# sukui-genomics-cn/hmm_layer

Hardware: AMD Instinct MI355X
Metric: HMM cell-updates/sec (batch x len x states) fwd-bwd, 15-state model (higher is better)
Workload: dtype f32

## Files before the change

### hmm_layer_amd/csrc/hmm_engine.hip

```cpp

#include <hip/hip_runtime.h>
#include <stdint.h>
#include <stdlib.h>
#include <mutex>
#include <type_traits>
#include <vector>
#include "hmm_engine.h"

typedef float f4 __attribute__((ext_vector_type(4)));
typedef int i4 __attribute__((ext_vector_type(4)));

#ifndef HMM_REDUCE_PF
#define HMM_REDUCE_PF 8
#endif
#ifndef HMM_NT_STORE
#define HMM_NT_STORE 1
#endif
#ifndef HMM_PSI
#define HMM_PSI 1
#endif
#ifndef HMM_BWD_FULL
#define HMM_BWD_FULL 0
#endif
#ifndef HMM_FWD_PF2
// ... 158 lines not shown
    f4 d = __builtin_amdgcn_mfma_f32_16x16x4f32(a[0], x.x, z, 0, 0, 0);
    d = __builtin_amdgcn_mfma_f32_16x16x4f32(a[1], x.y, d, 0, 0, 0);
    d = __builtin_amdgcn_mfma_f32_16x16x4f32(a[2], x.z, d, 0, 0, 0);
    d = __builtin_amdgcn_mfma_f32_16x16x4f32(a[3], x.w, d, 0, 0, 0);
    return d;
}

__device__ __forceinline__ f4 mfma4v(f4 a, f4 x, f4 c) {
    c = __builtin_amdgcn_mfma_f32_16x16x4f32(a.x, x.x, c, 0, 0, 0);
    c = __builtin_amdgcn_mfma_f32_16x16x4f32(a.y, x.y, c, 0, 0, 0);
    c = __builtin_amdgcn_mfma_f32_16x16x4f32(a.z, x.z, c, 0, 0, 0);
    c = __builtin_amdgcn_mfma_f32_16x16x4f32(a.w, x.w, c, 0, 0, 0);
    return c;
}

__device__ __forceinline__ void swap16(float &a, float &b) {
    asm("s_nop 1\n\tv_permlane16_swap_b32_e32 %0, %1" : "+v"(a), "+v"(b));
}
__device__ __forceinline__ void swap32(float &a, float &b) {
    asm("s_nop 1\n\tv_permlane32_swap_b32_e32 %0, %1" : "+v"(a), "+v"(b));
}
__device__ __forceinline__ float col_sum(float v) {
    float a = v, b = v;
    swap16(a, b);
    a += b; b = a;
    swap32(a, b);
    return a + b;
}
__device__ __forceinline__ float col_max(float v) {
    float a = v, b = v;
    swap16(a, b);
    a = fmaxf(a, b); b = a;
    swap32(a, b);
    return fmaxf(a, b);
}
__device__ __forceinline__ float hsum(f4 v) { return (v.x + v.y) + (v.z + v.w); }
__device__ __forceinline__ float hmax(f4 v) { return fmaxf(fmaxf(v.x, v.y), fmaxf(v.z, v.w)); }

__device__ __forceinline__ __amdgpu_buffer_rsrc_t make_rsrc(const void *base, unsigned long long bytes) {
    unsigned n = bytes > 0xFFFFFFF0ull ? 0xFFFFFFF0u : (unsigned)bytes;
    return __builtin_amdgcn_make_buffer_rsrc((void *)base, 0, (int)n, 0x00020000);
}
template <int N>
__device__ __forceinline__ void ld_rows(__amdgpu_buffer_rsrc_t r, int voff, int rowb, f4 (&e)[N]) {
#pragma unroll
    for (int s = 0; s < N; ++s)
        e[s] = __builtin_bit_cast(f4, __builtin_amdgcn_raw_buffer_load_b128(r, voff + s * rowb, 0, HMM_LD_AUX));
}

struct Bounds { f4 lo, hi; };
__device__ __forceinline__ Bounds make_bounds(int g, int q, float eps) {
    Bounds bd;
    const float inf = __builtin_inff();
    bd.lo.x = (4 * g + 0 < q) ? eps : 0.f;  bd.hi.x = (4 * g + 0 < q) ? inf : 0.f;
    bd.lo.y = (4 * g + 1 < q) ? eps : 0.f;  bd.hi.y = (4 * g + 1 < q) ? inf : 0.f;
    bd.lo.z = (4 * g + 2 < q) ? eps : 0.f;  bd.hi.z = (4 * g + 2 < q) ? inf : 0.f;
    bd.lo.w = (4 * g + 3 < q) ? eps : 0.f;  bd.hi.w = (4 * g + 3 < q) ? inf : 0.f;
    return bd;
}
__device__ __forceinline__ f4 clampE(f4 e, const Bounds &bd) {
    f4 r;
    r.x = __builtin_amdgcn_fmed3f(e.x, bd.lo.x, bd.hi.x);
    r.y = __builtin_amdgcn_fmed3f(e.y, bd.lo.y, bd.hi.y);
    r.z = __builtin_amdgcn_fmed3f(e.z, bd.lo.z, bd.hi.z);
    r.w = __builtin_amdgcn_fmed3f(e.w, bd.lo.w, bd.hi.w);
    return r;
}
__device__ __forceinline__ f4 fmax4(f4 v, float s) {
    f4 r = {fmaxf(v.x, s), fmaxf(v.y, s), fmaxf(v.z, s), fmaxf(v.w, s)};
    return r;
}
__device__ __forceinline__ f4 sel4(bool c, f4 a, f4 b) { return c ? a : b; }

__device__ __forceinline__ void load_A(const float *A, int q, int g, int n, float (&af)[4], float (&ab)[4]) {
#pragma unroll
    for (int kk = 0; kk < 4; ++kk) {
        int s = 4 * g + kk;
        bool ok = (s < q) && (n < q);
        af[kk] = ok ? A[s * q + n] : 0.f;
        ab[kk] = ok ? A[n * q + s] : 0.f;
    }
}


__device__ __forceinline__ void reduce_chain(const float *__restrict__ A, const float *__restrict__ E,
                                             float *__restrict__ ops, int *__restrict__ exps,
                                             const int *__restrict__ topo, const Plan &p, float eps, long long chain) {
    const int lane = threadIdx.x & 63, g = lane >> 4, n = lane & 15;
    const int seq = (int)(chain / p.C), c = (int)(chain - (long long)seq * p.C);
    const int m = seq / p.b;
    if (topo && topo[m] != 0) return;
    const int t0 = c * p.T;
    const int len = min(p.T, p.L - t0);
    const int q = p.q;

    float af[4], ab[4];
    load_A(A + (size_t)m * q * q, q, g, n, af, ab);
    const Bounds bd = make_bounds(g, q, eps);

    const float *base = E + ((size_t)seq * p.L + t0) * q;
    const __amdgpu_buffer_rsrc_t rs = make_rsrc(base, (unsigned long long)len * q * sizeof(float));
    const int rowb = q * (int)sizeof(float);
    int voff = g * 16;

    f4 X;
    X.x = (4 * g + 0 == n) ? 1.f : 0.f;
    X.y = (4 * g + 1 == n) ? 1.f : 0.f;
    X.z = (4 * g + 2 == n) ? 1.f : 0.f;
    X.w = (4 * g + 3 == n) ? 1.f : 0.f;
    int ex = 0;

    auto rescale = [&](f4 &V) {
        float s = col_sum(hsum(V));
        int xe = __builtin_amdgcn_frexp_expf(s);
        float sc = __builtin_amdgcn_ldexpf(1.0f, -xe);
        V = V * sc;
        ex += xe;
    };

    int t = 0;
    if (c == 0 && p.seq_start) {
        f4 e0[1];
        ld_rows<1>(rs, voff, rowb, e0);
        X = X * clampE(e0[0], bd);
        rescale(X);
        voff += rowb;
        t = 1;
    }
    constexpr int PF = HMM_REDUCE_PF;
    f4 en[PF];
    ld_rows<PF>(rs, voff, rowb, en);
    for (; t < len; t += PF) {
        f4 ec[PF];
#pragma unroll
        for (int u = 0; u < PF; ++u) ec[u] = en[u];
        voff += PF * rowb;
        ld_rows<PF>(rs, voff, rowb, en);
#pragma unroll
        for (int u = 0; u < PF; ++u) {
            if (t + u < len) {
                X = mfma4(af, X) * clampE(ec[u], bd);
                rescale(X);
            }
        }
    }
    float *o = ops + (size_t)chain * QP * QP;
    o[(4 * g + 0) * QP + n] = X.x;
    o[(4 * g + 1) * QP + n] = X.y;
    o[(4 * g + 2) * QP + n] = X.z;
    o[(4 * g + 3) * QP + n] = X.w;
    if (g == 0) exps[(size_t)chain * QP + n] = ex;
}

__global__ __launch_bounds__(256) void k_reduce(const float *__restrict__ A, const float *__restrict__ E,
                                                float *__restrict__ ops, int *__restrict__ exps,
                                                const int *__restrict__ topo, Plan p, float eps) {
    const long long stride = (long long)gridDim.x * 4;
    for (long long chain = (long long)blockIdx.x * 4 + __builtin_amdgcn_readfirstlane(threadIdx.x >> 6);
         chain < p.nchains; chain += stride)
        reduce_chain(A, E, ops, exps, topo, p, eps, chain);
}



struct TopoGene15 {
    static constexpr int Q = 15, NE = 23, ID = 1;
    static constexpr int start[Q + 1] = {0, 2, 4, 6, 8, 10, 13, 15, 16, 17, 18, 19, 20, 21, 22, 23};
    static constexpr int src[NE] = {0, 14, 8, 1, 9, 2, 10, 3, 11, 6, 7, 4, 12, 5, 13, 0, 4, 5, 6, 1, 2, 3, 5};
};
struct TopoGene7 {
    static constexpr int Q = 7, NE = 15, ID = 2;
    static constexpr int start[Q + 1] = {0, 2, 4, 6, 8, 11, 13, 15};
    static constexpr int src[NE] = {0, 6, 4, 1, 5, 2, 6, 3, 0, 6, 3, 4, 1, 5, 2};
};

struct TopoGene29 {
    static constexpr int Q = 29, NE = 45, ID = 3;
    static constexpr int start[Q + 1] = {0, 3, 5, 7, 9, 11, 13, 15, 17, 19, 22, 25, 27, 29, 30, 31, 32, 33, 34, 35, 36,
                                         37, 38, 39, 40, 41, 42, 43, 44, 45};
    static constexpr int src[NE] = {0, 27, 28, 15, 1, 16, 2, 17, 3, 18, 4, 19, 5, 20, 6, 21, 11, 22, 12, 13, 7, 23, 14,
                                    8, 24, 9, 25, 10, 26, 0, 0, 7, 8, 9, 10, 11, 12, 1, 2, 3, 4, 5, 6, 9, 10};
};

template <class T>
__host__ __device__ constexpr int out_degree(int i) {
    int n = 0;
    for (int e = 0; e < T::NE; ++e) n += (T::src[e] == i) ? 1 : 0;
    return n;
}
#define TOPO_UNIT 16
template <class T>
__host__ __device__ constexpr bool passthrough(int j) {
    return T::start[j + 1] - T::start[j] == 1 && out_degree<T>(j) == 1;
}
template <class T>
__host__ __device__ constexpr int pt_src(int p) { return T::src[T::start[p]]; }
template <class T>
__host__ __device__ constexpr int pt_dst(int p) {
    for (int j = 0; j < T::Q; ++j)
        for (int e = T::start[j]; e < T::start[j + 1]; ++e)
            if (T::src[e] == p) return j;
    return -1;
}
template <class T>
__host__ __device__ constexpr int n_passthrough() {
    int n = 0;
    for (int j = 0; j < T::Q; ++j) n += passthrough<T>(j) ? 1 : 0;
    return n;
}
template <class T>
__host__ __device__ constexpr bool passthrough_between_live() {
    for (int p = 0; p < T::Q; ++p)
        if (passthrough<T>(p) && (passthrough<T>(pt_src<T>(p)) || passthrough<T>(pt_dst<T>(p)))) return false;
    return true;
}
static_assert(n_passthrough<TopoGene15>() == 8 && passthrough_between_live<TopoGene15>(), "15-state gene model: 7 live states");
static_assert(n_passthrough<TopoGene29>() == 16 && passthrough_between_live<TopoGene29>(), "29-state gene model: 13 live states");
static_assert(n_passthrough<TopoGene7>() == 0, "the 7-state model has no pass-through state");
template <class T>
__device__ __forceinline__ bool edge_in(int i, int j) {
    bool ok = false;
    for (int e = T::start[j]; e < T::start[j + 1]; ++e) ok = ok || (T::src[e] == i);
    return ok;
}

#define TOPO_EXACT 255
__global__ __launch_bounds__(64) void k_topo_check(const float *__restrict__ A, int *__restrict__ topo, int k, int q,
                                                   int force_dense, int exact_mode, float eps, int *__restrict__ nexact,
                                                   int *__restrict__ wcnt = nullptr) {
    const int m = blockIdx.x;
    const float *Am = A + (size_t)m * q * q;
    if (m == 0 && threadIdx.x == 0) *nexact = 0;
    if (m == 0 && threadIdx.x < 4 && wcnt) wcnt[threadIdx.x] = 0;
    bool exact = exact_mode == HMM_EXACT_ALWAYS || exact_mode == HMM_EXACT_ALWAYS_NARROW;
    if (exact_mode == HMM_EXACT_AUTO) {
        int row = 0;
        if ((int)threadIdx.x < q)
            for (int j = 0; j < q; ++j) row |= (Am[threadIdx.x * q + j] > eps) ? (1 << j) : 0;
        for (int it = 0; it < 8; ++it) {
            int nr = 0;
            for (int j = 0; j < q; ++j) {
                const int rj = __builtin_amdgcn_readlane(row, j);
                nr |= ((row >> j) & 1) ? rj : 0;
            }
            row = nr;
        }
        const bool notfull = (int)threadIdx.x < q && row != (1 << q) - 1;
        exact = __ballot(notfull) != 0ull;
    }
    if (exact) {
        if (threadIdx.x == 0) topo[m] = TOPO_EXACT;
        return;
    }
    bool bad15 = q != TopoGene15::Q, bad7 = q != TopoGene7::Q;
    bool nonunit15 = false, nonunit7 = false;
    if (!force_dense && (!bad15 || !bad7))
        for (int e = threadIdx.x; e < q * q; e += 64) {
            const float a = Am[e];
            const int i = e / q, j = e - i * q;
            if (!bad15) {
                const bool in = edge_in<TopoGene15>(i, j);
                bad15 = a != 0.f && !in;
                nonunit15 = nonunit15 || (in && a != 1.0f && out_degree<TopoGene15>(i) == 1);
            }
            if (!bad7) {
                const bool in = edge_in<TopoGene7>(i, j);
                bad7 = a != 0.f && !in;
                nonunit7 = nonunit7 || (in && a != 1.0f && out_degree<TopoGene7>(i) == 1);
            }
        }
    const bool any15 = __ballot(bad15) != 0ull, any7 = __ballot(bad7) != 0ull;
    const bool nu15 = __ballot(nonunit15) != 0ull, nu7 = __ballot(nonunit7) != 0ull;
    if (threadIdx.x == 0) {
        int id = force_dense ? 0 : (!any15 ? TopoGene15::ID : (!any7 ? TopoGene7::ID : 0));
        if (id == TopoGene15::ID && !nu15) id |= TOPO_UNIT;
        if (id == TopoGene7::ID && !nu7) id |= TOPO_UNIT;
        topo[m] = id;
    }
}

#define SP_TILE 16

#ifndef HMM_RS_AHEAD
#define HMM_RS_AHEAD 0
#endif
#ifndef HMM_RS_UNI
#define HMM_RS_UNI 1
#endif
#ifndef HMM_POST_BLOCK
#define HMM_POST_BLOCK 16
#endif
#ifndef HMM_RS_SUM2
#define HMM_RS_SUM2 1
#endif
#ifndef HMM_RS_ORDER2
#define HMM_RS_ORDER2 1
#endif
#ifndef HMM_RS_ROW128
#define HMM_RS_ROW128 1
#endif
#ifndef HMM_RS_WPE
#define HMM_RS_WPE 4
#endif
#if HMM_RS_WPE
#define RS_ATTR __attribute__((amdgpu_waves_per_eu(HMM_RS_WPE, HMM_RS_WPE)))
#else
#define RS_ATTR
#endif
template <class T> struct RsCfg {
    static constexpr int W = T::Q <= 16 ? 16 : 32;
    static constexpr int CPW = 64 / W;
    static constexpr int PIECES = SP_TILE * T::Q / 4;
    static constexpr int RPC = (PIECES + 63) / 64;
    typedef float Lds[2][CPW][SP_TILE * W + 16];
};

template <class T, bool UNIT, bool UNI>
__device__ __forceinline__ void reduce_sparse_wave(const float *__restrict__ A, const float *__restrict__ E,
                                                   float *__restrict__ ops, int *__restrict__ exps, const Plan &p,
                                                   float eps, typename RsCfg<T>::Lds &ldsw, long long wchain0,
                                                   bool mine, int m, long long chain, int c) {
    constexpr int Q = T::Q, W = RsCfg<T>::W, CPW = RsCfg<T>::CPW, RPC = RsCfg<T>::RPC;
    constexpr bool O2 = HMM_RS_ORDER2 && UNIT && UNI && n_passthrough<T>() > 0;
    static_assert(!O2 || passthrough_between_live<T>(), "a pass-through state between two live states");
    auto live = [](int j) constexpr { return !O2 || !passthrough<T>(j); };
    const int lane = threadIdx.x & 63, cl = lane / W, kc = lane % W;
    const int t0 = c * p.T;
    const int len = mine ? min(p.T, p.L - t0) : 0;
    const bool first = (c == 0) && p.seq_start;

    float a[T::NE];
    {
        const float *Am = A + (size_t)(UNI ? __builtin_amdgcn_readfirstlane(m) : m) * Q * Q;
#pragma unroll
        for (int j = 0; j < Q; ++j)
#pragma unroll
            for (int e = T::start[j]; e < T::start[j + 1]; ++e) a[e] = Am[T::src[e] * Q + j];
    }

    const int seq0 = (int)(wchain0 / p.C), c0 = (int)(wchain0 - (long long)seq0 * p.C);
    const long long row0 = (long long)seq0 * p.L + (long long)c0 * p.T;
    const unsigned long long total = (unsigned long long)p.NB * p.L * Q * sizeof(float);
    const __amdgpu_buffer_rsrc_t rs = make_rsrc(E + row0 * Q, total - (unsigned long long)row0 * Q * sizeof(float));
    constexpr int PIECES = RsCfg<T>::PIECES;
    static_assert(SP_TILE * Q % 4 == 0, "tile must be a whole number of 16-byte pieces");
    int coff[CPW];
#pragma unroll
    for (int j = 0; j < CPW; ++j) {
        long long ch = wchain0 + j;
        if (ch >= p.nchains) ch = wchain0;
        const long long sq = ch / p.C;
        const long long rw = sq * p.L + (ch - sq * p.C) * (long long)p.T;
        coff[j] = (int)((rw - row0) * Q * (long long)sizeof(float));
    }
    int loff[RPC][4];
#pragma unroll
    for (int rr = 0; rr < RPC; ++rr)
#pragma unroll
        for (int u = 0; u < 4; ++u) {
            const int idx = 4 * (rr * 64 + lane) + u;
            loff[rr][u] = (idx / Q) * W + (idx % Q);
        }
    float smul[O2 ? RPC : 1][4];
    if constexpr (O2) {
#pragma unroll
        for (int rr = 0; rr < RPC; ++rr)
#pragma unroll
            for (int u = 0; u < 4; ++u) {
                const int st = (4 * (rr * 64 + lane) + u) % Q;
                float mv = 1.f;
#pragma unroll
                for (int pp = 0; pp < Q; ++pp)
                    if (passthrough<T>(pp)) mv = (st == pp) ? a[T::start[pp]] : mv;
                smul[rr][u] = mv;
            }
    }
    for (int i = lane; i < 2 * CPW * (SP_TILE * W + 16); i += 64) (&ldsw[0][0][0])[i] = 0.f;

    f4 r[CPW * RPC];
    auto fetch = [&](int tile) {
#pragma unroll
        for (int j = 0; j < CPW; ++j)
#pragma unroll
            for (int rr = 0; rr < RPC; ++rr)
                r[j * RPC + rr] = __builtin_bit_cast(f4, __builtin_amdgcn_raw_buffer_load_b128(
                    rs, coff[j] + tile * (SP_TILE * Q * 4) + (rr * 64 + lane) * 16, 0, 0));
    };
    auto stage = [&](int buf) {
#pragma unroll
        for (int rr = 0; rr < RPC; ++rr) {
            if (rr * 64 + lane < PIECES) {
#pragma unroll
                for (int j = 0; j < CPW; ++j) {
                    float *dst = &ldsw[buf][j][0];
                    const f4 v = r[j * RPC + rr];
                    if constexpr (O2) {
                        dst[loff[rr][0]] = fmaxf(v.x, eps) * smul[rr][0];
                        dst[loff[rr][1]] = fmaxf(v.y, eps) * smul[rr][1];
                        dst[loff[rr][2]] = fmaxf(v.z, eps) * smul[rr][2];
                        dst[loff[rr][3]] = fmaxf(v.w, eps) * smul[rr][3];
                    } else {
                        dst[loff[rr][0]] = fmaxf(v.x, eps);
                        dst[loff[rr][1]] = fmaxf(v.y, eps);
                        dst[loff[rr][2]] = fmaxf(v.z, eps);
                        dst[loff[rr][3]] = fmaxf(v.w, eps);
                    }
                }
            }
        }
    };

    float x[Q], pend[Q], xb[O2 ? Q : 1];
    auto flight_src = [&](int i) {
        bool f = false;
#pragma unroll
        for (int pp = 0; pp < Q; ++pp)
            if (passthrough<T>(pp) && pt_src<T>(pp) == i) f = f || (kc == pp);
        return f;
    };
#pragma unroll
    for (int j = 0; j < Q; ++j) {
        x[j] = (j == kc) ? 1.f : 0.f;
        pend[j] = 1.f;
        if constexpr (O2) {
            pend[j] = x[j];
            xb[j] = flight_src(j) ? 1.f : 0.f;
        }
    }
    int ex = 0;
    float cs = (kc < Q) ? 1.f : 0.f;
    auto deferred = [](int j) constexpr { return !O2 && UNIT && out_degree<T>(j) == 1; };

    bool risk = false;
    auto rescale = [&]() {
        risk = risk || (kc < Q && cs < 0x1p-100f);
        int xe = max(__builtin_amdgcn_frexp_expf(cs), -100);
        float sc = __builtin_amdgcn_ldexpf(1.0f, -xe);
#pragma unroll
        for (int j = 0; j < Q; ++j) {
            if (live(j)) x[j] *= sc;
            if constexpr (O2) { if (live(j)) xb[j] *= sc; }
        }
        cs *= sc;
        ex += xe;
    };

    auto entry = [&](int j) {
        if constexpr (O2) return live(j) ? x[j] : pend[j] * xb[pt_src<T>(j)];
        else return deferred(j) ? x[j] * pend[j] : x[j];
    };
    auto column_sum = [&]() {
        float s = 0.f;
        if constexpr (O2) {
#pragma unroll
            for (int j = 0; j < Q; ++j) if (live(j)) s += x[j];
#pragma unroll
            for (int j = 0; j < Q; ++j) if (!live(j)) s = fmaf(pend[j], xb[pt_src<T>(j)], s);
        } else {
#pragma unroll
            for (int j = 0; j < Q; ++j) s += entry(j);
        }
        return s;
    };
    auto finish = [&]() {
        cs = kc < Q ? column_sum() : 0.f;
        rescale();
        float *o = ops + (size_t)chain * W * W;
#pragma unroll
        for (int j = 0; j < Q; ++j) o[j * W + kc] = (kc < Q) ? entry(j) : 0.f;
#pragma unroll
        for (int j = Q; j < W; ++j) o[j * W + kc] = 0.f;
        static_assert(Q < W, "the exponent row's last lane is a pad lane");
        const unsigned long long rb = __builtin_amdgcn_ballot_w64(risk) >> (W == 64 ? 0 : W * cl);
        const bool chain_risk = (W == 64 ? rb : (rb & ((1ull << (W & 63)) - 1ull))) != 0ull;
        exps[(size_t)chain * W + kc] = (kc < Q) ? ex : ((kc == W - 1 && chain_risk) ? 1 : 0);
    };
    auto step = [&](const float (&e)[Q], auto sumc) {
        constexpr bool SUM = decltype(sumc)::value;
        float y[Q];
        float s = 0.f;
        if constexpr (O2) {
#pragma unroll
            for (int j = 0; j < Q; ++j) {
                if (!live(j)) continue;
                float acc = 0.f;
                bool any = false;
#pragma unroll
                for (int pass = 0; pass < 2; ++pass)
#pragma unroll
                    for (int ed = T::start[j]; ed < T::start[j + 1]; ++ed) {
                        const int i = T::src[ed];
                        if (live(i) != (pass == 0)) continue;
                        const float w = live(i) ? a[ed] : pend[i];
                        const float v = live(i) ? x[i] : xb[pt_src<T>(i)];
                        acc = any ? fmaf(w, v, acc) : w * v;
                        any = true;
                    }
                y[j] = acc;
            }
#pragma unroll
            for (int j = 0; j < Q; ++j) {
                if (live(j)) { xb[j] = x[j]; x[j] = y[j] * e[j]; }
                else pend[j] = e[j];
            }
            if (SUM) s = column_sum();
        } else {
#pragma unroll
            for (int j = 0; j < Q; ++j) {
                float acc = 0.f;
#pragma unroll
                for (int ed = T::start[j]; ed < T::start[j + 1]; ++ed) {
                    const int i = T::src[ed];
                    const float w = deferred(i) ? pend[i] : a[ed];
                    acc = (ed == T::start[j]) ? w * x[i] : fmaf(w, x[i], acc);
                }
                y[j] = acc;
            }
#pragma unroll
            for (int j = 0; j < Q; ++j) {
                if (SUM) s = fmaf(y[j], e[j], s);
                if (deferred(j)) { x[j] = y[j]; pend[j] = e[j]; }
                else x[j] = y[j] * e[j];
            }
        }
        if (SUM) {
            if (W >= 32) {
                const unsigned long long keep = __builtin_amdgcn_ballot_w64(kc < Q && !(s < cs * 0x1p-45f));
                const unsigned long long mine = W == 64 ? ~0ull : (((1ull << (W & 63)) - 1ull) << (W * cl));
                risk = risk || (keep & mine) == 0ull;
            }
            cs = s;
            const unsigned cb = __builtin_bit_cast(unsigned, cs) - 1u;
            if (__builtin_amdgcn_ballot_w64(cb < 0x2B800000u - 1u) != 0) rescale();
        }
    };

    auto ldrow = [&](const float *rowp, float (&r)[Q]) {
#pragma unroll
        for (int v = 0; v + 4 <= Q; v += 4) {
            const f4 t = *reinterpret_cast<const f4 *>(rowp + v);
            r[v] = t.x; r[v + 1] = t.y; r[v + 2] = t.z; r[v + 3] = t.w;
        }
        constexpr int R0 = Q & ~3;
        if constexpr (Q - R0 == 3 && HMM_RS_ROW128) {
            static_assert(R0 + 4 <= W, "the pad float belongs to the row");
            const f4 t = *reinterpret_cast<const f4 *>(rowp + R0);
            r[R0] = t.x; r[R0 + 1] = t.y; r[R0 + 2] = t.z;
        } else if constexpr (Q - R0 == 3) {
            typedef float f3 __attribute__((ext_vector_type(3)));
            const f3 t = *reinterpret_cast<const f3 *>(rowp + R0);
            r[R0] = t.x; r[R0 + 1] = t.y; r[R0 + 2] = t.z;
        } else if constexpr (Q - R0 == 2) {
            typedef float f2 __attribute__((ext_vector_type(2)));
            const f2 t = *reinterpret_cast<const f2 *>(rowp + R0);
            r[R0] = t.x; r[R0 + 1] = t.y;
        } else if constexpr (Q - R0 == 1) {
            r[R0] = rowp[R0];
        }
    };

    const int ntiles = p.T / SP_TILE;
    const int last = len - 1;
    const bool ragged = __builtin_amdgcn_ballot_w64(mine && len != p.T) != 0;
    auto tile_steps = [&](auto checked, int tile, int buf) {
        constexpr bool CHECK = decltype(checked)::value;
        const float *tp = &ldsw[buf][cl][0];
        constexpr bool AHEAD = W == 16 && HMM_RS_AHEAD;
        float c[Q], nx[AHEAD ? Q : 1];
        ldrow(tp, c);
        if constexpr (AHEAD) ldrow(tp + W, nx);
        if (tile == 0) {
            float xs[Q];
#pragma unroll
            for (int j = 0; j < Q; ++j) xs[j] = O2 ? (j == kc ? 1.f : 0.f) : x[j];
            float e0 = 1.f;
            if constexpr (O2) { if (first && mine && kc < Q) e0 = fmaxf(E[(chain / p.C) * (long long)p.L * Q + kc], eps); }
            step(c, std::true_type());
            if (first) {
                if constexpr (!O2) e0 = tp[kc < Q ? kc : 0];
#pragma unroll
                for (int j = 0; j < Q; ++j) {
                    x[j] = xs[j] * e0;
                    pend[j] = 1.f;
                    if constexpr (O2) { pend[j] = x[j]; xb[j] = flight_src(j) ? 1.f : 0.f; }
                }
                cs = (kc < Q) ? e0 : 0.f;
                ex = 0;
                rescale();
            }
        } else {
            step(c, std::integral_constant<bool, !HMM_RS_SUM2>());
        }
        if (CHECK) { if (__builtin_amdgcn_ballot_w64(tile * SP_TILE == last) != 0) { if (tile * SP_TILE == last) finish(); } }
        auto one = [&](int sidx, auto sumc) {
            if constexpr (AHEAD) {
#pragma unroll
                for (int u = 0; u < Q; ++u) c[u] = nx[u];
                if (sidx + 1 < SP_TILE) ldrow(tp + (sidx + 1) * W, nx);
            } else {
                ldrow(tp + sidx * W, c);
            }
            step(c, sumc);
            if (CHECK) {
                const int t = tile * SP_TILE + sidx;
                if (__builtin_amdgcn_ballot_w64(t == last) != 0) { if (t == last) finish(); }
            }
        };
#pragma unroll
        for (int sidx = 1; sidx < SP_TILE; sidx += 2) {
            one(sidx, std::true_type());
            if (sidx + 1 < SP_TILE) one(sidx + 1, std::integral_constant<bool, !HMM_RS_SUM2>());
        }
    };
    fetch(0);
    if (ragged) {
        for (int tile = 0; tile < ntiles; ++tile) {
            stage(tile & 1);
            if (tile + 1 < ntiles) fetch(tile + 1);
            tile_steps(std::true_type(), tile, tile & 1);
        }
    } else {
        for (int tile = 0; tile < ntiles; ++tile) {
            stage(tile & 1);
            if (tile + 1 < ntiles) fetch(tile + 1);
            tile_steps(std::false_type(), tile, tile & 1);
        }
        if (mine) finish();
    }
}

template <class T, bool MIXED>
__device__ __forceinline__ void reduce_sparse_block(const float *__restrict__ A, const float *__restrict__ E,
                                                    float *__restrict__ ops, int *__restrict__ exps,
                                                    const int *__restrict__ topo, const Plan &p, float eps) {
    __shared__ __attribute__((aligned(16))) typename RsCfg<T>::Lds lds[4];
    const int w = __builtin_amdgcn_readfirstlane(threadIdx.x >> 6);
    const int lane = threadIdx.x & 63, cl = lane / RsCfg<T>::W;
    const long long wchain0 = ((long long)blockIdx.x * 4 + w) * RsCfg<T>::CPW;
    if (wchain0 >= p.nchains) return;
    const long long chain = wchain0 + cl;
    const bool inrange = chain < p.nchains;
    const long long chn = inrange ? chain : wchain0;
    const int seq = (int)(chn / p.C), c = (int)(chn - (long long)seq * p.C);
    const int m = seq / p.b;
    const int tp = topo[m];
    const bool mine = inrange && (tp & (TOPO_UNIT - 1)) == T::ID && tp != TOPO_EXACT;
    const unsigned long long mmask = __builtin_amdgcn_ballot_w64(mine);
    if (mmask == 0) return;
    const bool unit = __builtin_amdgcn_ballot_w64(mine && (tp & TOPO_UNIT)) == mmask;
    const bool uni = HMM_RS_UNI && __builtin_amdgcn_ballot_w64(m != __builtin_amdgcn_readfirstlane(m)) == 0ull;
    if (uni == MIXED) return;
    if (unit) reduce_sparse_wave<T, true, !MIXED>(A, E, ops, exps, p, eps, lds[w], wchain0, mine, m, chain, c);
    else reduce_sparse_wave<T, false, !MIXED>(A, E, ops, exps, p, eps, lds[w], wchain0, mine, m, chain, c);
}

template <class T, bool MIXED = false>
__global__ __launch_bounds__(256) RS_ATTR void k_reduce_sparse(const float *__restrict__ A, const float *__restrict__ E,
                                                       float *__restrict__ ops, int *__restrict__ exps,
                                                       const int *__restrict__ topo, Plan p, float eps) {
    reduce_sparse_block<T, MIXED>(A, E, ops, exps, topo, p, eps);
}
template <class T, bool MIXED = false>
__global__ __launch_bounds__(256) void k_reduce_sparse_wide(const float *__restrict__ A, const float *__restrict__ E,
                                                            float *__restrict__ ops, int *__restrict__ exps,
                                                            const int *__restrict__ topo, Plan p, float eps) {
    reduce_sparse_block<T, MIXED>(A, E, ops, exps, topo, p, eps);
}


template <class Op>
__device__ __forceinline__ int row_allreduce_i(int v, Op op) {
    v = op(v, __builtin_amdgcn_update_dpp(v, v, 0xB1, 0xF, 0xF, false));
    v = op(v, __builtin_amdgcn_update_dpp(v, v, 0x4E, 0xF, 0xF, false));
    v = op(v, __builtin_amdgcn_update_dpp(v, v, 0x141, 0xF, 0xF, false));
    v = op(v, __builtin_amdgcn_update_dpp(v, v, 0x140, 0xF, 0xF, false));
    return v;
}
__device__ __forceinline__ float row_sum_f(float x) {
    int v = __builtin_bit_cast(int, x);
    auto add = [](int a, int b) { return __builtin_bit_cast(int, __builtin_bit_cast(float, a) + __builtin_bit_cast(float, b)); };
    return __builtin_bit_cast(float, row_allreduce_i(v, add));
}
__device__ __forceinline__ int row_max_i(int x) {
    return row_allreduce_i(x, [](int a, int b) { return a > b ? a : b; });
}
__device__ __forceinline__ float lane_bcast(float x, int srclane) {
    return __builtin_bit_cast(float, __builtin_amdgcn_readlane(__builtin_bit_cast(int, x), srclane));
}
template <int K>
__device__ __forceinline__ float row_bcast_f(float x) {
    return __builtin_bit_cast(float, __builtin_amdgcn_update_dpp(0, __builtin_bit_cast(int, x), 0x150 + K, 0xF, 0xF, false));
}
__device__ __forceinline__ float row_dot16(const float (&c)[16], float v) {
    float a0 = 0.f, a1 = 0.f;
    a0 = fmaf(c[0], row_bcast_f<0>(v), a0);   a1 = fmaf(c[1], row_bcast_f<1>(v), a1);
    a0 = fmaf(c[2], row_bcast_f<2>(v), a0);   a1 = fmaf(c[3], row_bcast_f<3>(v), a1);
    a0 = fmaf(c[4], row_bcast_f<4>(v), a0);   a1 = fmaf(c[5], row_bcast_f<5>(v), a1);
    a0 = fmaf(c[6], row_bcast_f<6>(v), a0);   a1 = fmaf(c[7], row_bcast_f<7>(v), a1);
    a0 = fmaf(c[8], row_bcast_f<8>(v), a0);   a1 = fmaf(c[9], row_bcast_f<9>(v), a1);
    a0 = fmaf(c[10], row_bcast_f<10>(v), a0); a1 = fmaf(c[11], row_bcast_f<11>(v), a1);
    a0 = fmaf(c[12], row_bcast_f<12>(v), a0); a1 = fmaf(c[13], row_bcast_f<13>(v), a1);
    a0 = fmaf(c[14], row_bcast_f<14>(v), a0); a1 = fmaf(c[15], row_bcast_f<15>(v), a1);
    return a0 + a1;
}

__global__ __launch_bounds__(128) void k_scan(const float *__restrict__ pi, const float *__restrict__ ops,
                                             const int *__restrict__ exps, float *__restrict__ prefix,
                                             double *__restrict__ llpre, float *__restrict__ suffix,
                                             double *__restrict__ lsuf, double *__restrict__ loglik,
                                             const int *__restrict__ topo, Plan p, float eps,
                                             const float *__restrict__ pre_in = nullptr,
                                             const double *__restrict__ ll_in = nullptr,
                                             const float *__restrict__ suf_in = nullptr,
                                             const double *__restrict__ ls_in = nullptr) {
    const int seq = blockIdx.x;
    const int lane = threadIdx.x & 63;
    const int dir = __builtin_amdgcn_readfirstlane(threadIdx.x >> 6);
    const int n = lane & 15;
    const int q = p.q, C = p.C;
    const int m = seq / p.b;
    const size_t chain0 = (size_t)seq * C;
    if (lane >= 16) return;
    if (topo[m] == TOPO_EXACT) return;
    if (dir == 0) {
        float praw = pre_in ? pre_in[(size_t)seq * QP + n] : ((n < q) ? pi[(size_t)m * q + n] : 0.f);
        float a = pre_in ? praw : ((n < q) ? fmaxf(praw, eps) : 0.f);
        double ll = ll_in ? ll_in[seq] : 0.0;
        prefix[chain0 * QP + n] = praw;
        if (n == 0) llpre[chain0] = ll;
        const f4 *row = reinterpret_cast<const f4 *>(ops + chain0 * QP * QP + n * QP);
        f4 r0 = row[0], r1 = row[1], r2 = row[2], r3 = row[3];
        int xe = exps[chain0 * QP + n];
        for (int c = 0; c < C; ++c) {
            const f4 q0 = r0, q1 = r1, q2 = r2, q3 = r3;
            const int xec = xe;
            if (c + 1 < C) {
                const f4 *nx = reinterpret_cast<const f4 *>(ops + (chain0 + c + 1) * QP * QP + n * QP);
                r0 = nx[0]; r1 = nx[1]; r2 = nx[2]; r3 = nx[3];
                xe = exps[(chain0 + c + 1) * QP + n];
            }
            int we = (a > 0.f) ? __builtin_amdgcn_frexp_expf(a) + xec : -(1 << 28);
            const int emax = row_max_i(we);
            int sh = xec - emax;
            sh = sh < -300 ? -300 : sh;
            float w = __builtin_amdgcn_ldexpf(a, sh);
            float acc = 0.f;
            float xr[16] = {q0.x, q0.y, q0.z, q0.w, q1.x, q1.y, q1.z, q1.w, q2.x, q2.y, q2.z, q2.w, q3.x, q3.y, q3.z, q3.w};
#pragma unroll
            for (int kk = 0; kk < 16; ++kk) acc = fmaf(xr[kk], lane_bcast(w, kk), acc);
            const float S = row_sum_f(acc);
            a = acc / S;
            ll += (double)__logf(S) + (double)emax * LN2;
            if (c + 1 < C) {
                prefix[(chain0 + c + 1) * QP + n] = a;
                if (n == 0) llpre[chain0 + c + 1] = ll;
            }
        }
        if (n == 0) loglik[seq] = ll;
    } else {
        float v = suf_in ? suf_in[(size_t)seq * QP + n] : ((n < q) ? 1.f : 0.f);
        double lb = ls_in ? ls_in[seq] : 0.0;
        float col[16];
        int xe = 0;
        if (C > 1) {
            const float *X = ops + (chain0 + C - 1) * QP * QP;
#pragma unroll
            for (int j = 0; j < 16; ++j) col[j] = X[j * QP + n];
            xe = exps[(chain0 + C - 1) * QP + n];
        }
        for (int c = C - 1; c >= 0; --c) {
            suffix[(chain0 + c) * QP + n] = v;
            if (n == 0) lsuf[chain0 + c] = lb;
            if (c == 0) break;
            float cc[16];
#pragma unroll
            for (int j = 0; j < 16; ++j) cc[j] = col[j];
            const int xec = xe;
            if (c - 1 > 0) {
                const float *X = ops + (chain0 + c - 1) * QP * QP;
#pragma unroll
                for (int j = 0; j < 16; ++j) col[j] = X[j * QP + n];
                xe = exps[(chain0 + c - 1) * QP + n];
            }
            float u = 0.f;
#pragma unroll
            for (int j = 0; j < 16; ++j) u = fmaf(cc[j], lane_bcast(v, j), u);
            int we = (u > 0.f) ? __builtin_amdgcn_frexp_expf(u) + xec : -(1 << 28);
            const int emax = row_max_i(we);
            int sh = xec - emax;
            sh = sh < -300 ? -300 : sh;
            v = __builtin_amdgcn_ldexpf(u, sh);
            lb += (double)emax * LN2;
        }
    }
}

__device__ __forceinline__ int col_max_i(int v) {
    float a = __builtin_bit_cast(float, v), b2 = a;
    swap16(a, b2);
    v = max(__builtin_bit_cast(int, a), __builtin_bit_cast(int, b2));
    a = __builtin_bit_cast(float, v); b2 = a;
    swap32(a, b2);
    return max(__builtin_bit_cast(int, a), __builtin_bit_cast(int, b2));
}

__global__ __launch_bounds__(256) void k_scan_compose(const float *__restrict__ ops, const int *__restrict__ exps,
                                                      float *__restrict__ gops, int *__restrict__ gexps,
                                                      const int *__restrict__ topo, Plan p) {
    const long long wv = (long long)blockIdx.x * 4 + __builtin_amdgcn_readfirstlane(threadIdx.x >> 6);
    if (wv >= (long long)p.NB * p.G) return;
    const int lane = threadIdx.x & 63, g = lane >> 4, n = lane & 15;
    const int seq = (int)(wv / p.G), grp = (int)(wv - (long long)seq * p.G);
    if (topo[seq / p.b] == TOPO_EXACT) return;
    const int c0 = grp * p.gsize, c1 = min(p.C, c0 + p.gsize);
    f4 X = {4 * g + 0 == n ? 1.f : 0.f, 4 * g + 1 == n ? 1.f : 0.f, 4 * g + 2 == n ? 1.f : 0.f, 4 * g + 3 == n ? 1.f : 0.f};
    int ex = 0;
    const size_t chb = (size_t)seq * p.C;
    f4 an[SCAN_PF];
    i4 en[SCAN_PF];
#pragma unroll
    for (int u = 0; u < SCAN_PF; ++u) {
        const int c = min(c0 + u, c1 - 1);
        an[u] = *reinterpret_cast<const f4 *>(ops + (chb + c) * QP * QP + n * QP + 4 * g);
        en[u] = *reinterpret_cast<const i4 *>(exps + (chb + c) * QP + 4 * g);
    }
    for (int cb = c0; cb < c1; cb += SCAN_PF)
#pragma unroll
      for (int u = 0; u < SCAN_PF; ++u) {
        const int c = cb + u;
        if (c >= c1) break;
        const f4 a4 = an[u];
        const i4 e4 = en[u];
        if (c + SCAN_PF < c1) {
            an[u] = *reinterpret_cast<const f4 *>(ops + (chb + c + SCAN_PF) * QP * QP + n * QP + 4 * g);
            en[u] = *reinterpret_cast<const i4 *>(exps + (chb + c + SCAN_PF) * QP + 4 * g);
        }
        int we = -(1 << 28);
        we = X.x > 0.f ? max(we, __builtin_amdgcn_frexp_expf(X.x) + e4.x) : we;
        we = X.y > 0.f ? max(we, __builtin_amdgcn_frexp_expf(X.y) + e4.y) : we;
        we = X.z > 0.f ? max(we, __builtin_amdgcn_frexp_expf(X.z) + e4.z) : we;
        we = X.w > 0.f ? max(we, __builtin_amdgcn_frexp_expf(X.w) + e4.w) : we;
        const int emax = col_max_i(we);
        f4 W;
        W.x = __builtin_amdgcn_ldexpf(X.x, max(e4.x - emax, -300));
        W.y = __builtin_amdgcn_ldexpf(X.y, max(e4.y - emax, -300));
        W.z = __builtin_amdgcn_ldexpf(X.z, max(e4.z - emax, -300));
        W.w = __builtin_amdgcn_ldexpf(X.w, max(e4.w - emax, -300));
        const float af[4] = {a4.x, a4.y, a4.z, a4.w};
        X = mfma4(af, W);
        const float sden = col_sum(hsum(X));
        const int xe = __builtin_amdgcn_frexp_expf(sden);
        X = X * __builtin_amdgcn_ldexpf(1.0f, -xe);
        ex += emax + xe;
    }
    float *o = gops + (size_t)wv * QP * QP;
    o[(4 * g + 0) * QP + n] = X.x;
    o[(4 * g + 1) * QP + n] = X.y;
    o[(4 * g + 2) * QP + n] = X.z;
    o[(4 * g + 3) * QP + n] = X.w;
    if (g == 0) gexps[(size_t)wv * QP + n] = ex;
}

__global__ __launch_bounds__(128) void k_scan_inner(const float *__restrict__ ops, const int *__restrict__ exps,
                                                   const float *__restrict__ gprefix, const double *__restrict__ gllpre,
                                                   const float *__restrict__ gsuffix, const double *__restrict__ glsuf,
                                                   float *__restrict__ prefix, double *__restrict__ llpre,
                                                   float *__restrict__ suffix, double *__restrict__ lsuf,
                                                   const int *__restrict__ topo, Plan p, float eps) {
    const int lane = threadIdx.x & 63;
    const int dir = __builtin_amdgcn_readfirstlane(threadIdx.x >> 6);
    const int n = lane & 15;
    const int q = p.q;
    const long long blk = (long long)blockIdx.x * 4 + (lane >> 4);
    bool valid = blk < (long long)p.NB * p.G;
    const long long bl = valid ? blk : 0;
    const int seq = (int)(bl / p.G), grp = (int)(bl - (long long)seq * p.G);
    valid = valid && topo[seq / p.b] != TOPO_EXACT;
    const int c0 = grp * p.gsize, c1 = min(p.C, c0 + p.gsize);
    const size_t chain0 = (size_t)seq * p.C;
    int hops = valid ? c1 - 1 - c0 : 0;
    for (int o = 32; o > 0; o >>= 1) hops = max(hops, __shfl_xor(hops, o));
    if (dir == 0) {
        const float pin = valid ? gprefix[(size_t)bl * QP + n] : 0.f;
        float a = (grp == 0 && p.seq_start) ? ((n < q) ? fmaxf(pin, eps) : 0.f) : pin;
        double ll = valid ? gllpre[bl] : 0.0;
        if (valid) {
            prefix[(chain0 + c0) * QP + n] = pin;
            if (n == 0) llpre[chain0 + c0] = ll;
        }
        float rw[SCAN_PF][16];
        int xe[SCAN_PF];
        auto fetch = [&](int u, int c) {
            const f4 *row = reinterpret_cast<const f4 *>(ops + (chain0 + c) * QP * QP + n * QP);
            const f4 r0 = row[0], r1 = row[1], r2 = row[2], r3 = row[3];
            rw[u][0] = r0.x; rw[u][1] = r0.y; rw[u][2] = r0.z; rw[u][3] = r0.w; rw[u][4] = r1.x; rw[u][5] = r1.y;
            rw[u][6] = r1.z; rw[u][7] = r1.w; rw[u][8] = r2.x; rw[u][9] = r2.y; rw[u][10] = r2.z; rw[u][11] = r2.w;
            rw[u][12] = r3.x; rw[u][13] = r3.y; rw[u][14] = r3.z; rw[u][15] = r3.w;
            xe[u] = exps[(chain0 + c) * QP + n];
        };
#pragma unroll
        for (int u = 0; u < SCAN_PF; ++u) {
            xe[u] = 0;
#pragma unroll
            for (int k = 0; k < 16; ++k) rw[u][k] = 0.f;
            if (valid && c0 + u + 1 < c1) fetch(u, c0 + u);
        }
        for (int hb = 0; hb < hops; hb += SCAN_PF)
#pragma unroll
          for (int u = 0; u < SCAN_PF; ++u) {
            const int h = hb + u;
            if (h >= hops) break;
            const int c = c0 + h;
            const bool on = valid && c + 1 < c1;
            float cur[16];
#pragma unroll
            for (int k = 0; k < 16; ++k) cur[k] = rw[u][k];
            const int xec = xe[u];
            if (valid && c + SCAN_PF + 1 < c1) fetch(u, c + SCAN_PF);
            int we = (a > 0.f) ? __builtin_amdgcn_frexp_expf(a) + xec : -(1 << 28);
            const int emax = row_max_i(we);
            int sh = xec - emax;
            sh = sh < -300 ? -300 : sh;
            const float w = __builtin_amdgcn_ldexpf(a, sh);
            const float acc = row_dot16(cur, w);
            const float S = row_sum_f(acc);
            if (on) {
                a = acc / S;
                ll += (double)__logf(S) + (double)emax * LN2;
                prefix[(chain0 + c + 1) * QP + n] = a;
                if (n == 0) llpre[chain0 + c + 1] = ll;
            }
// ... 1481 lines not shown
```

Baseline: 262.6 billion.

## Split ragged tail tile out of sparse reduce loop and single-buffer LDS

The sparse reduce wave loop no longer checks per step whether the current step is a chain's last one on ragged inputs. Full tiles run unchecked up to the tile holding the last chain's end. That one tile runs in a non-unrolled loop that calls finish at the cut, and the remaining tiles run unchecked. The LDS tile buffer drops from two to one by default, which halves shared memory per wave and may raise occupancy. An optional two-deep register prefetch is added but off by default. With one LDS buffer, staging the next tile can overwrite data other lanes are still reading unless wave-level ordering covers it.

```diff
diff --git a/hmm_layer_amd/csrc/hmm_engine.hip b/hmm_layer_amd/csrc/hmm_engine.hip
--- a/hmm_layer_amd/csrc/hmm_engine.hip
+++ b/hmm_layer_amd/csrc/hmm_engine.hip
@@ -484,6 +484,15 @@
 #ifndef HMM_RS_WPE
 #define HMM_RS_WPE 4
 #endif
+#ifndef HMM_RS_TAIL2
+#define HMM_RS_TAIL2 1
+#endif
+#ifndef HMM_RS_LDSBUF
+#define HMM_RS_LDSBUF 1
+#endif
+#ifndef HMM_RS_PF2
+#define HMM_RS_PF2 0
+#endif
 #if HMM_RS_WPE
 #define RS_ATTR __attribute__((amdgpu_waves_per_eu(HMM_RS_WPE, HMM_RS_WPE)))
 #else
@@ -494,7 +503,10 @@
     static constexpr int CPW = 64 / W;
     static constexpr int PIECES = SP_TILE * T::Q / 4;
     static constexpr int RPC = (PIECES + 63) / 64;
-    typedef float Lds[2][CPW][SP_TILE * W + 16];
+    static constexpr int NBUF = HMM_RS_LDSBUF;
+    static constexpr int DEPTH = (W == 16 && HMM_RS_PF2) ? 2 : 1;
+    static_assert(NBUF == 1 || NBUF == 2, "HMM_RS_LDSBUF: one or two tile buffers");
+    typedef float Lds[NBUF][CPW][SP_TILE * W + 16];
 };
 
 template <class T, bool UNIT, bool UNI>
@@ -557,25 +569,28 @@
                 smul[rr][u] = mv;
             }
     }
-    for (int i = lane; i < 2 * CPW * (SP_TILE * W + 16); i += 64) (&ldsw[0][0][0])[i] = 0.f;
-
-    f4 r[CPW * RPC];
-    auto fetch = [&](int tile) {
+    constexpr int NBUF = RsCfg<T>::NBUF, DEPTH = RsCfg<T>::DEPTH;
+    for (int i = lane; i < NBUF * CPW * (SP_TILE * W + 16); i += 64) (&ldsw[0][0][0])[i] = 0.f;
+
+    f4 r[DEPTH][CPW * RPC];
+    auto fetch = [&](int tile, auto slotc) {
+        constexpr int SLOT = decltype(slotc)::value;
 #pragma unroll
         for (int j = 0; j < CPW; ++j)
 #pragma unroll
             for (int rr = 0; rr < RPC; ++rr)
-                r[j * RPC + rr] = __builtin_bit_cast(f4, __builtin_amdgcn_raw_buffer_load_b128(
+                r[SLOT][j * RPC + rr] = __builtin_bit_cast(f4, __builtin_amdgcn_raw_buffer_load_b128(
                     rs, coff[j] + tile * (SP_TILE * Q * 4) + (rr * 64 + lane) * 16, 0, 0));
     };
-    auto stage = [&](int buf) {
+    auto stage = [&](int buf, auto slotc) {
+        constexpr int SLOT = decltype(slotc)::value;
 #pragma unroll
         for (int rr = 0; rr < RPC; ++rr) {
             if (rr * 64 + lane < PIECES) {
 #pragma unroll
                 for (int j = 0; j < CPW; ++j) {
                     float *dst = &ldsw[buf][j][0];
-                    const f4 v = r[j * RPC + rr];
+                    const f4 v = r[SLOT][j * RPC + rr];
                     if constexpr (O2) {
                         dst[loff[rr][0]] = fmaxf(v.x, eps) * smul[rr][0];
                         dst[loff[rr][1]] = fmaxf(v.y, eps) * smul[rr][1];
@@ -742,15 +757,8 @@
     };
 
     const int ntiles = p.T / SP_TILE;
-    const int last = len - 1;
     const bool ragged = __builtin_amdgcn_ballot_w64(mine && len != p.T) != 0;
-    auto tile_steps = [&](auto checked, int tile, int buf) {
-        constexpr bool CHECK = decltype(checked)::value;
-        const float *tp = &ldsw[buf][cl][0];
-        constexpr bool AHEAD = W == 16 && HMM_RS_AHEAD;
-        float c[Q], nx[AHEAD ? Q : 1];
-        ldrow(tp, c);
-        if constexpr (AHEAD) ldrow(tp + W, nx);
+    auto head = [&](const float (&c)[Q], int tile, const float *tp) {
         if (tile == 0) {
             float xs[Q];
 #pragma unroll
@@ -773,7 +781,21 @@
         } else {
             step(c, std::integral_constant<bool, !HMM_RS_SUM2>());
         }
+    };
+#if !HMM_RS_TAIL2
+    const int last = len - 1;
+#endif
+    auto tile_steps = [&](auto checked, int tile, int buf) {
+        constexpr bool CHECK = decltype(checked)::value;
+        const float *tp = &ldsw[buf][cl][0];
+        constexpr bool AHEAD = W == 16 && HMM_RS_AHEAD;
+        float c[Q], nx[AHEAD ? Q : 1];
+        ldrow(tp, c);
+        if constexpr (AHEAD) ldrow(tp + W, nx);
+        head(c, tile, tp);
+#if !HMM_RS_TAIL2
         if (CHECK) { if (__builtin_amdgcn_ballot_w64(tile * SP_TILE == last) != 0) { if (tile * SP_TILE == last) finish(); } }
+#endif
         auto one = [&](int sidx, auto sumc) {
             if constexpr (AHEAD) {
 #pragma unroll
@@ -783,10 +805,12 @@
                 ldrow(tp + sidx * W, c);
             }
             step(c, sumc);
+#if !HMM_RS_TAIL2
             if (CHECK) {
                 const int t = tile * SP_TILE + sidx;
                 if (__builtin_amdgcn_ballot_w64(t == last) != 0) { if (t == last) finish(); }
             }
+#endif
         };
 #pragma unroll
         for (int sidx = 1; sidx < SP_TILE; sidx += 2) {
@@ -794,21 +818,66 @@
             if (sidx + 1 < SP_TILE) one(sidx + 1, std::integral_constant<bool, !HMM_RS_SUM2>());
         }
     };
-    fetch(0);
+    typedef std::integral_constant<int, 0> Slot0;
+#if HMM_RS_TAIL2
+    typedef std::integral_constant<int, DEPTH - 1> Slot1;
+    auto buf_of = [](int tile) { return NBUF == 2 ? (tile & 1) : 0; };
+    auto stage_tile = [&](int tile) {
+        if (DEPTH == 2 && (tile & 1)) stage(buf_of(tile), Slot1());
+        else stage(buf_of(tile), Slot0());
+    };
+    auto refill = [&](int tile) {
+        if (tile + DEPTH >= ntiles) return;
+        if (DEPTH == 2 && (tile & 1)) fetch(tile + DEPTH, Slot1());
+        else fetch(tile + DEPTH, Slot0());
+    };
+    auto run_tiles = [&](int lo, int hi) {
+        for (int tile = lo; tile < hi; ++tile) {
+            stage_tile(tile);
+            refill(tile);
+            tile_steps(std::false_type(), tile, buf_of(tile));
+        }
+    };
+    const int ltail = p.L - (p.C - 1) * p.T;
+    const int cut_tile = ragged ? (ltail - 1) / SP_TILE : ntiles;
+    fetch(0, Slot0());
+    if constexpr (DEPTH == 2) { if (1 < ntiles) fetch(1, Slot1()); }
+    run_tiles(0, cut_tile);
+    if (ragged) {
+        const int cut = ltail - cut_tile * SP_TILE;
+        const float *tp = &ldsw[buf_of(cut_tile)][cl][0];
+        stage_tile(cut_tile);
+#pragma nounroll
+        for (int sidx = 0; sidx < SP_TILE; ++sidx) {
+            float c[Q];
+            ldrow(tp + sidx * W, c);
+            if (sidx == 0) head(c, cut_tile, tp);
+            else if (sidx & 1) step(c, std::true_type());
+            else step(c, std::integral_constant<bool, !HMM_RS_SUM2>());
+            if (sidx + 1 == cut) { if (mine && len != p.T) finish(); }
+        }
+        refill(cut_tile);
+        run_tiles(cut_tile + 1, ntiles);
+    }
+    if (mine && len == p.T) finish();
+#else
+    static_assert(DEPTH == 1, "HMM_RS_PF2 needs HMM_RS_TAIL2");
+    fetch(0, Slot0());
     if (ragged) {
         for (int tile = 0; tile < ntiles; ++tile) {
-            stage(tile & 1);
-            if (tile + 1 < ntiles) fetch(tile + 1);
-            tile_steps(std::true_type(), tile, tile & 1);
+            stage(NBUF == 2 ? (tile & 1) : 0, Slot0());
+            if (tile + 1 < ntiles) fetch(tile + 1, Slot0());
+            tile_steps(std::true_type(), tile, NBUF == 2 ? (tile & 1) : 0);
         }
     } else {
         for (int tile = 0; tile < ntiles; ++tile) {
-            stage(tile & 1);
-            if (tile + 1 < ntiles) fetch(tile + 1);
-            tile_steps(std::false_type(), tile, tile & 1);
+            stage(NBUF == 2 ? (tile & 1) : 0, Slot0());
+            if (tile + 1 < ntiles) fetch(tile + 1, Slot0());
+            tile_steps(std::false_type(), tile, NBUF == 2 ? (tile & 1) : 0);
         }
         if (mine) finish();
     }
+#endif
 }
 
 template <class T, bool MIXED>
```

Result: no change. 261.3 billion (-0.5%).
